# fu5ha/rayn

Measured on NVIDIA H100. Metric: Msamples/sec (pixels x spp), higher is better.
Workload: dtype f32

## Files before the change

rayn_b200/csrc/rt_kernels.cuh:

```cuda
#pragma once
#include "rt_device.cuh"
#include "rt_sdf2.cuh"

namespace rt {

struct DevFrame {
  int W, H, tile_w, tile_h, samples, spp, max_bounces, vm;
  int ntx, nty, sets_1d, sets_2d;
  float t0, t1;
  const float* __restrict__ s1;
  const float* __restrict__ s2;
  const float* __restrict__ scramble;
  const float* __restrict__ fis;
};

struct PassBufs {
  int n_tiles;
  int R;
  int QS;
  const int* __restrict__ tile_ids;
  float4* o_time;
  float4* d_t;
  float4* rad;
  float4* thr;
// ... 82 lines not shown
    }
  }
  *closest = c;
  *id = best;
}

__global__ void __launch_bounds__(256) k_raygen(const __grid_constant__ DevScene sc, const DevFrame fr, const PassBufs pb, const int pre_n) {
  const int ts = blockIdx.y;
  const int i = blockIdx.x * blockDim.x + threadIdx.x;
  const TileGeom tg = tile_geom(fr, pb.tile_ids[ts]);
  if (i == 0) pb.n_live[ts] = tg.npaths;
  if (i >= tg.npaths) return;
  const int pl = i / fr.spp, s = i - pl * fr.spp;
  const int xl = pl / tg.th, yl = pl - xl * tg.th;
  const int x = tg.x0 + xl, y = tg.y0 + yl;
  const float scramble = __ldg(fr.scramble + x + (size_t)y * fr.W);
  const float fx = fis_sample(fr.fis, samp2(fr, 0, s, scramble, 0));
  const float fy = fis_sample(fr.fis, samp2(fr, 1, s, scramble, 0));
  const float sx = ((float)x + 0.5f) + fx;
  const float sy = ((float)y + 0.5f) + fy;
  const float u = (1.0f / (float)fr.W) * sx;
  const float v = (1.0f / (float)fr.H) * sy;
  const float time = fr.t0 + (fr.t1 - fr.t0) * samp1(fr, s, scramble, 0);
  const float ls0 = samp2(fr, 0, s, scramble, 1), ls1 = samp2(fr, 1, s, scramble, 1);
  const float time0 = fr.t0 + (fr.t1 - fr.t0) * samp1(fr, s & ~3, scramble, 0);
  f3 ro, rd;
  camera_ray(sc.cam, u, v, ls0, ls1, time0, &ro, &rd);
  const size_t g = (size_t)ts * pb.R + i;
  float closest = 0.0f;
  int hit_id = -1;
  if (pre_n >= 0) fold_head(sc, pre_n, ro, rd, &closest, &hit_id);
  pb.o_time[g] = make_float4(ro.x, ro.y, ro.z, time);
  pb.d_t[g] = make_float4(rd.x, rd.y, rd.z, closest);
  pb.q_key[g] = hit_id;
  pb.rad[g] = make_float4(0.0f, 0.0f, 0.0f, 0.0f);
  pb.thr[g] = make_float4(1.0f, 1.0f, 1.0f, 0.0f);
  pb.nrm0[g] = make_float4(0.0f, 0.0f, 0.0f, __uint_as_float(0u));
  pb.term[g] = 0u;
  pb.q_live[g] = i;
}

#define BIN_T 1024
#define SEG_SLOTS 32768
__global__ void __launch_bounds__(BIN_T) k_bin_count(const PassBufs pb, const int n_hit, const int nseg) {
  const int seg = blockIdx.x, ts = blockIdx.y, tid = threadIdx.x, lane = tid & 31;
  const int n = pb.n_live[ts];
  __shared__ int cnt[RAYN_MAX_HITABLES];
  const int* __restrict__ qk = pb.q_key + (size_t)ts * pb.R;
  const int* __restrict__ ql = pb.q_live + (size_t)ts * pb.R;
  if (tid < RAYN_MAX_HITABLES) cnt[tid] = 0;
  if (tid == 0 && seg == 0 && n) atomicAdd(pb.counters + CNT_EXTEND_RAYS, (unsigned long long)n);
  __syncthreads();
  const int lo = seg * SEG_SLOTS, hi = min(n, lo + SEG_SLOTS);
  for (int base = lo; base < hi; base += BIN_T) {
    const int i = base + tid;
    const int key = i < hi ? qk[ql[i]] : -1;
    const unsigned m = __match_any_sync(0xffffffffu, key);
    if (key >= 0 && (m & ((1u << lane) - 1)) == 0) atomicAdd(&cnt[key], __popc(m));
  }
  __syncthreads();
  if (tid < n_hit) pb.seg_cnt[((size_t)ts * nseg + seg) * RAYN_MAX_HITABLES + tid] = cnt[tid];
}
__global__ void __launch_bounds__(BIN_T) k_bin_scatter(const PassBufs pb, const int n_hit, const int nseg) {
  const int seg = blockIdx.x, ts = blockIdx.y, tid = threadIdx.x, lane = tid & 31, warp = tid >> 5;
  constexpr int NW = BIN_T / 32;
  const int n = pb.n_live[ts];
  const int lo = seg * SEG_SLOTS, hi = min(n, lo + SEG_SLOTS);
  if (lo >= n && seg > 0) return;
  __shared__ int cnt[RAYN_MAX_HITABLES];
  __shared__ int before[RAYN_MAX_HITABLES];
  __shared__ int start[RAYN_MAX_HITABLES + 1];
  __shared__ int running[2][RAYN_MAX_HITABLES];
  __shared__ int wcnt[2][NW][RAYN_MAX_HITABLES];
  const int* __restrict__ qk = pb.q_key + (size_t)ts * pb.R;
  const int* __restrict__ ql = pb.q_live + (size_t)ts * pb.R;
  int* __restrict__ qs = pb.q_shade + (size_t)ts * pb.QS;
  if (tid < n_hit) {
    const int used = (n + SEG_SLOTS - 1) / SEG_SLOTS;
    int tot = 0, bef = 0;
    for (int sg = 0; sg < used; ++sg) {
      const int c = pb.seg_cnt[((size_t)ts * nseg + sg) * RAYN_MAX_HITABLES + tid];
      if (sg < seg) bef += c;
      tot += c;
    }
    cnt[tid] = tot, before[tid] = bef;
  }
  __syncthreads();
  if (tid == 0) {
    int off = 0;
    for (int o = 0; o < n_hit; ++o) {
      start[o] = off;
      running[0][o] = off + before[o];
      off += (cnt[o] + 3) & ~3;
    }
    start[n_hit] = off;
    if (seg == 0) pb.n_slots[ts] = off;
  }
  __syncthreads();
  if (seg == 0 && tid <= n_hit) pb.bin_start[ts * (RAYN_MAX_HITABLES + 1) + tid] = start[tid];
  int buf = 0;
  for (int base = lo; base < hi; base += BIN_T, buf ^= 1) {
    const int i = base + tid;
    const int id = i < hi ? ql[i] : -1;
    const int key = i < hi ? qk[id] : -1;
    unsigned mine = 0;
    for (int k = 0; k < n_hit; ++k) {
      const unsigned b = __ballot_sync(0xffffffffu, key == k);
      if (key == k) mine = b;
      if (lane == k) wcnt[buf][warp][k] = __popc(b);
    }
    __syncthreads();
    if (key >= 0) {
      int off = running[buf][key] + __popc(mine & ((1u << lane) - 1));
      for (int w = 0; w < warp; ++w) off += wcnt[buf][w][key];
      qs[off] = id;
    }
    if (tid < n_hit) {
      int tot = running[buf][tid];
      for (int w = 0; w < NW; ++w) tot += wcnt[buf][w][tid];
      running[buf ^ 1][tid] = tot;
    }
  }
  if (seg == 0 && tid < n_hit)
    for (int k = start[tid] + cnt[tid]; k < start[tid + 1]; ++k) qs[k] = -1;
}

#define EXT_BATCH 128
#define SCAN_T 1024
__global__ void __launch_bounds__(SCAN_T) k_scan_live(const PassBufs pb, int* __restrict__ batch_prefix, int* __restrict__ work_ctr) {
  __shared__ int wsum[SCAN_T / 32];
  __shared__ int carry;
  const int tid = threadIdx.x, lane = tid & 31, warp = tid >> 5;
  if (tid == 0) {
    carry = 0;
  }
  if (tid < WC_TOTAL) work_ctr[tid] = 0;
  __syncthreads();
  for (int base = 0; base < pb.n_tiles; base += SCAN_T) {
    const int i = base + tid;
    const int v = i < pb.n_tiles ? (pb.n_live[i] + EXT_BATCH - 1) / EXT_BATCH : 0;
    int x = v;
    for (int o = 1; o < 32; o <<= 1) {
      const int y = __shfl_up_sync(0xffffffffu, x, o);
      if (lane >= o) x += y;
    }
    if (lane == 31) wsum[warp] = x;
    __syncthreads();
    if (warp == 0) {
      int w = wsum[lane];
      for (int o = 1; o < 32; o <<= 1) {
        const int y = __shfl_up_sync(0xffffffffu, w, o);
        if (lane >= o) w += y;
      }
      wsum[lane] = w;
    }
    __syncthreads();
    const int excl = carry + (warp ? wsum[warp - 1] : 0) + x - v;
    if (i < pb.n_tiles) batch_prefix[i] = excl;
    __syncthreads();
    if (tid == SCAN_T - 1) carry = excl + v;
    __syncthreads();
  }
  if (tid == 0) batch_prefix[pb.n_tiles] = carry;
}

#define SLOT_BLOCK 128
__global__ void __launch_bounds__(SCAN_T) k_scan_slots(const __grid_constant__ DevScene sc, const PassBufs pb) {
  __shared__ int wsum[SCAN_T / 32];
  __shared__ int carry;
  const int tid = threadIdx.x, lane = tid & 31, warp = tid >> 5;
  for (int row = 0; row <= sc.n_sdf; ++row) {
    int* __restrict__ out = pb.slot_prefix + (size_t)row * pb.prefix_stride;
    const int hk = row ? sc.sdf_idx[row - 1] : 0;
    if (tid == 0) carry = 0;
    __syncthreads();
    for (int base = 0; base < pb.n_tiles; base += SCAN_T) {
      const int i = base + tid;
      int v = 0;
      if (i < pb.n_tiles) {
        const int* __restrict__ bs = pb.bin_start + i * (RAYN_MAX_HITABLES + 1);
        const int slots = row ? bs[hk + 1] - bs[hk] : pb.n_slots[i];
        v = (slots + SLOT_BLOCK - 1) / SLOT_BLOCK;
      }
      int x = v;
      for (int o = 1; o < 32; o <<= 1) {
        const int y = __shfl_up_sync(0xffffffffu, x, o);
        if (lane >= o) x += y;
      }
      if (lane == 31) wsum[warp] = x;
      __syncthreads();
      if (warp == 0) {
        int w = wsum[lane];
        for (int o = 1; o < 32; o <<= 1) {
          const int y = __shfl_up_sync(0xffffffffu, w, o);
          if (lane >= o) w += y;
        }
        wsum[lane] = w;
      }
      __syncthreads();
      const int excl = carry + (warp ? wsum[warp - 1] : 0) + x - v;
      if (i < pb.n_tiles) out[i] = excl;
      __syncthreads();
      if (tid == SCAN_T - 1) carry = excl + v;
      __syncthreads();
    }
    if (tid == 0) out[pb.n_tiles] = carry;
    __syncthreads();
  }
}
#define WORK_CHUNK 8
RT_D int grab_chunk(int* __restrict__ ctr, int* s_slot) {
  if (threadIdx.x == 0) *s_slot = atomicAdd(ctr, WORK_CHUNK);
  __syncthreads();
  const int c = *s_slot;
  __syncthreads();
  return c;
}
RT_D int find_tile(const int* __restrict__ prefix, int n_tiles, int wb) {
  int lo = 0, hi = n_tiles;
  while (hi - lo > 1) {
    const int mid = (lo + hi) >> 1;
    if (__ldg(prefix + mid) <= wb) lo = mid; else hi = mid;
  }
  return lo;
}
#define FOR_EACH_WORK_BLOCK(prefix, n_tiles, ctr, ...)                                  \
  {                                                                                     \
    __shared__ int s_chunk_;                                                            \
    const int total_ = (prefix)[n_tiles];                                               \
    for (;;) {                                                                          \
      const int c0_ = grab_chunk(ctr, &s_chunk_);                                       \
      if (c0_ >= total_) break;                                                         \
      const int c1_ = min(c0_ + WORK_CHUNK, total_);                                    \
      int ts = 0, begin_ = 0, end_ = 0;                                                 \
      for (int wb_ = c0_; wb_ < c1_; ++wb_) {                                           \
        if (wb_ >= end_) {                                                              \
          ts = find_tile(prefix, n_tiles, wb_);                                         \
          begin_ = __ldg((prefix) + ts), end_ = __ldg((prefix) + ts + 1);               \
        }                                                                               \
        const int local = wb_ - begin_;                                                 \
        __VA_ARGS__                                                                     \
      }                                                                                 \
    }                                                                                   \
  }

__global__ void __launch_bounds__(EXT_BATCH) k_extend_spheres(const __grid_constant__ DevScene sc, const PassBufs pb, const int first, const int last,
                                                              const int init, const int moving, const int* __restrict__ batch_prefix,
                                                              int* __restrict__ work_ctr) {
  FOR_EACH_WORK_BLOCK(batch_prefix, pb.n_tiles, work_ctr, {
    const int i = local * EXT_BATCH + threadIdx.x;
    const int n = pb.n_live[ts];
    if (i < n) {
      const size_t q = (size_t)ts * pb.R + i;
      const size_t g = (size_t)ts * pb.R + pb.q_live[q];
      const float4 o4 = pb.o_time[g], d4 = pb.d_t[g];
      const f3 o = mk3(o4.x, o4.y, o4.z), d = mk3(d4.x, d4.y, d4.z);
      float closest = init ? sc.rc.world_radius * 2.0f : d4.w;
      int id = init ? -1 : pb.q_key[g];
      float time0 = o4.w;
      if (moving && (i & 3)) time0 = pb.o_time[(size_t)ts * pb.R + pb.q_live[(size_t)ts * pb.R + (i & ~3)]].w;
      for (int k = first; k < last; ++k) {
        const float t = moving ? sphere_hit(sc.hit[k], o, d, closest, time0) : sphere_hit_static(sc.sph[sc.hit_ord[k]], o, d, closest);
        if (t < closest) {
          closest = t;
          id = k;
        }
      }
      pb.d_t[g].w = closest;
      pb.q_key[g] = id;
    }
  })
}

#define EXT_T 128
#ifndef RAYN_MARCH_OCC
#define RAYN_MARCH_OCC 8
#endif
#ifndef RAYN_MARCH_OCC_BULB
#define RAYN_MARCH_OCC_BULB RAYN_MARCH_OCC
#endif
#define MARCH_OCC(V) ((V) == SDFV_BULB ? RAYN_MARCH_OCC_BULB : RAYN_MARCH_OCC)
struct MarchSlot {
  float ox, oy, oz, dx, dy, dz;
  float px, py, pz;
  float t, t_max;
  int id, steps;
};
RT_D void slot_start(MarchSlot& s, float4 o, float4 d, float t_max) {
  s.ox = o.x, s.oy = o.y, s.oz = o.z, s.dx = d.x, s.dy = d.y, s.dz = d.z;
  s.px = o.x, s.py = o.y, s.pz = o.z;
  s.t = -0.0f, s.t_max = t_max, s.steps = -1;
}
RT_D void slot_advance(MarchSlot& s) {
  s.px = dm::mul_add(s.dx, s.t, s.ox), s.py = dm::mul_add(s.dy, s.t, s.oy), s.pz = dm::mul_add(s.dz, s.t, s.oz);
}
RT_D void slot_park(MarchSlot& s) { s.px = 100.0f, s.py = 0.0f, s.pz = 0.0f; }
RT_D MarchSlot slot_empty() {
  MarchSlot s;
  slot_start(s, make_float4(0.0f, 0.0f, 0.0f, 0.0f), make_float4(0.0f, 0.0f, 0.0f, 0.0f), 0.0f);
  s.id = -1;
  return s;
}

template <bool THR_CONST>
RT_D bool extend_step(MarchSlot& s, float d, float c0, float c1, float thr_scale, int max_marches, bool* hit) {
  const float th = THR_CONST ? c1 : __fmul_rn(c1, __fmul_rn(thr_scale, s.t));
  const float ad = dm::abs(d);
  const bool h = (s.steps >= 0) && ((ad < c0) || (ad < th));
  const float tn = __fadd_rn(s.t, d);
  const int sn = s.steps + 1;
  s.t = h ? s.t : tn;
  s.steps = h ? s.steps : sn;
  *hit = h;
  return h | (tn != tn) | (sn >= max_marches) | (tn > s.t_max);
}

template <int V, bool THR_CONST>
__global__ void __launch_bounds__(EXT_T, MARCH_OCC(V)) k_extend_march(const __grid_constant__ DevScene sc, const PassBufs pb, const Thr thr,
                                                          const int hk, const int spheres_first, const int* __restrict__ batch_prefix,
                                                          int* __restrict__ work_ctr) {
  const SdfK k = make_sdfk(sc.hit[hk]);
  const int lane = threadIdx.x & 31;
  const unsigned lt = (1u << lane) - 1u;
  const float S = sc.rc.sdf_detail_scale;
  const float c0 = 0.00005f * S;
  const float c1 = THR_CONST ? (0.05f * S) * thr.scale : 0.05f * S;
  const int max_marches = sc.rc.max_marches;
  const int n_batches = batch_prefix[pb.n_tiles];
  MarchSlot s0 = slot_empty(), s1 = slot_empty();
  int evals = 0, bulb_iters = 0, trips = 0;
  int cur_base = 0, cur_pos = 0, cur_end = 0;
  bool exhausted = false;
  while (true) {
    if (!exhausted) {
      unsigned idle0 = __ballot_sync(0xffffffffu, s0.id < 0), idle1 = __ballot_sync(0xffffffffu, s1.id < 0);
      while (idle0 | idle1) {
        if (cur_pos >= cur_end) {
          int b = 0;
          if (lane == 0) b = atomicAdd(work_ctr, 1);
          b = __shfl_sync(0xffffffffu, b, 0);
          if (b >= n_batches) {
            exhausted = true;
            break;
          }
          int lo = 0, hi = pb.n_tiles;
          while (hi - lo > 1) {
            const int mid = (lo + hi) >> 1;
            if (__ldg(batch_prefix + mid) <= b) lo = mid; else hi = mid;
          }
          cur_base = lo * pb.R;
          cur_pos = (b - __ldg(batch_prefix + lo)) * EXT_BATCH;
          cur_end = min(cur_pos + EXT_BATCH, pb.n_live[lo]);
        }
        const int avail = cur_end - cur_pos;
        const int n0 = __popc(idle0);
        const int rank0 = __popc(idle0 & lt), rank1 = n0 + __popc(idle1 & lt);
        if (s0.id < 0 && rank0 < avail) {
          const int g = cur_base + pb.q_live[cur_base + cur_pos + rank0];
          const float4 d4 = pb.d_t[g];
          slot_start(s0, pb.o_time[g], d4, d4.w);
          s0.id = g;
        }
        if (s1.id < 0 && rank1 < avail) {
          const int g = cur_base + pb.q_live[cur_base + cur_pos + rank1];
          const float4 d4 = pb.d_t[g];
          slot_start(s1, pb.o_time[g], d4, d4.w);
          s1.id = g;
        }
        cur_pos += min(avail, n0 + __popc(idle1));
        idle0 = __ballot_sync(0xffffffffu, s0.id < 0), idle1 = __ballot_sync(0xffffffffu, s1.id < 0);
      }
    }
    if (exhausted) {
      if (!__any_sync(0xffffffffu, s0.id >= 0 || s1.id >= 0)) break;
      if (s0.id < 0) slot_park(s0);
      if (s1.id < 0) slot_park(s1);
    }
    const float2 dd = sdf_dist2<V>(k, f2(s0.px, s1.px), f2(s0.py, s1.py), f2(s0.pz, s1.pz), bulb_iters);
    ++trips;
    bool hit0, hit1;
    const bool done0 = extend_step<THR_CONST>(s0, dd.x, c0, c1, thr.scale, max_marches, &hit0);
    const bool done1 = extend_step<THR_CONST>(s1, dd.y, c0, c1, thr.scale, max_marches, &hit1);
    slot_advance(s0);
    slot_advance(s1);
    if (done0 | done1) {
      if (done0 && s0.id >= 0) {
        if (s0.t < s0.t_max || (spheres_first && s0.t == s0.t_max && pb.q_key[s0.id] > hk)) {
          pb.d_t[s0.id].w = s0.t;
          pb.q_key[s0.id] = hk;
        }
        evals += s0.steps + (hit0 ? 2 : 1);
        s0.id = -1;
      }
      if (done1 && s1.id >= 0) {
        if (s1.t < s1.t_max || (spheres_first && s1.t == s1.t_max && pb.q_key[s1.id] > hk)) {
          pb.d_t[s1.id].w = s1.t;
          pb.q_key[s1.id] = hk;
        }
        evals += s1.steps + (hit1 ? 2 : 1);
        s1.id = -1;
      }
    }
  }
  warp_add(pb.counters + CNT_EVALS_EXTEND, evals);
  if (lane == 0) atomicAdd(pb.counters + CNT_TRIPS_EXTEND, (unsigned long long)trips);
  if (V == SDFV_BULB) warp_add(pb.counters + CNT_BULB_ITERS_EXTEND, bulb_iters);
}

template <int V, bool TRAP>
__global__ void __launch_bounds__(128, 8) k_normals(const __grid_constant__ DevScene sc, const PassBufs pb, const Thr thr, const int hk, const int j,
                                                    int* __restrict__ work_ctr) {
  const int* __restrict__ prefix = pb.slot_prefix + (size_t)(1 + j) * pb.prefix_stride;
  const SdfK k = make_sdfk(sc.hit[hk]);
  int evals = 0;
  FOR_EACH_WORK_BLOCK(prefix, pb.n_tiles, work_ctr, {
    const int* __restrict__ bs = pb.bin_start + ts * (RAYN_MAX_HITABLES + 1);
    const int s = bs[hk] + local * SLOT_BLOCK + threadIdx.x;
    const int id = s < bs[hk + 1] ? pb.q_shade[(size_t)ts * pb.QS + s] : -1;
    if (id >= 0) {
      const size_t g = (size_t)ts * pb.R + id;
      const float4 o4 = pb.o_time[g], d4 = pb.d_t[g];
      const f3 point = fma3s(mk3(d4.x, d4.y, d4.z), d4.w, mk3(o4.x, o4.y, o4.z));
      const float eps = dm::max(0.0001f, sc.rc.sdf_detail_scale * thr.at(d4.w));
      int it = 0;
      const float ex = 1.0f * eps, en = -1.0f * eps;
      const float2 da = sdf_dist2<V>(k, f2(point.x + ex, point.x + en), f2(point.y + en, point.y + en), f2(point.z + en, point.z + ex), it);
      const float2 db = sdf_dist2<V>(k, f2(point.x + en, point.x + ex), f2(point.y + ex, point.y + ex), f2(point.z + en, point.z + ex), it);
      f3 n = mk3(1.0f, -1.0f, -1.0f) * da.x;
      n = n + mk3(-1.0f, -1.0f, 1.0f) * da.y;
      n = n + mk3(-1.0f, 1.0f, -1.0f) * db.x;
      n = n + mk3(1.0f, 1.0f, 1.0f) * db.y;
      n = normalized(n);
      pb.nrm[g] = make_float4(n.x, n.y, n.z, eps);
      evals += 4;
      if (TRAP) pb.trap_s[g] = trap_coord(sc.trap[sc.hit[hk].material], sdf_trap(sc.hit[hk], point));
    }
  })
  warp_add(pb.counters + CNT_EVALS_NORMALS, evals);
}
struct LightContrib {
  f3 start, end_point, c;
  float den, trans;
};
RT_D LightContrib light_contrib(const RaynLight& L, const RaynMaterial& mat, f3 albedo, const ShadingPoint& sp, f3 wo, int round, float u0,
                                float u1, float vol_sample, bool has_ext, float neg_rho_t) {
  LightContrib r;
  f3 li;
  r.trans = 1.0f;
  if (round == 0) {
    float pdf;
    light_sample(L, u0, u1, sp.point, &r.end_point, &li, &pdf);
    f3 wi = r.end_point - sp.point;
    const float dist = mag(wi);
    wi = wi / dist;
    r.start = sp.point + sp.normal * dm::signum(dot(sp.normal, wi)) * sp.offset_by;
    const f3 f = bsdf_f(mat, albedo, wo, wi, sp.normal) * dm::max(dot(sp.normal, wi), 0.0f);
    const float tr = has_ext ? dm::exp(neg_rho_t * dist) : 1.0f;
    r.c = li * f * tr;
    r.den = pdf;
  } else {
    float vol_dist, vol_pdf, light_pdf;
    light_sample_volume(L, vol_sample, sp.o, sp.d, sp.t, &vol_dist, &vol_pdf);
    r.start = sp.o + sp.d * vol_dist;
    light_sample(L, u0, u1, r.start, &r.end_point, &li, &light_pdf);
    const float dist_point_to_light = mag(r.end_point - r.start);
    const float f = 1.0f / (4.0f * RT_PI);
    const float tr = has_ext ? dm::exp(neg_rho_t * dist_point_to_light) : 1.0f;
    r.c = li * f * tr;
    r.den = vol_pdf * light_pdf;
    r.trans = has_ext ? dm::exp(neg_rho_t * vol_dist) : 1.0f;
  }
  return r;
}

RT_D f3 hit_albedo(const DevScene& sc, const PassBufs& pb, const RaynHitable& h, const RaynMaterial& mat, size_t g) {
  if (sc.trap_mask != 0u && ((sc.trap_mask >> h.material) & 1u))
    return trap_albedo(sc.trap[h.material], h.kind == RAYN_HITABLE_SPHERE ? 1.0f : pb.trap_s[g]);
  return ld3(mat.albedo);
}

struct SlotCtx {
  int id, sample, obj;
  float scramble;
  unsigned w0, w1, w2;
  int set1, set2;
};
RT_D SlotCtx slot_ctx(const DevScene& sc, const DevFrame& fr, const PassBufs& pb, int ts, int s, int nslots, int depth, int lane) {
  SlotCtx c;
  const int* __restrict__ qs = pb.q_shade + (size_t)ts * pb.QS;
  c.id = s < nslots ? qs[s] : -1;
  c.sample = 0;
  c.obj = 0;
  c.scramble = 0.0f;
  if (c.id >= 0) {
    c.obj = pb.q_key[(size_t)ts * pb.R + c.id];
    const TileGeom tg = tile_geom(fr, pb.tile_ids[ts]);
    const int pl = c.id / fr.spp;
    c.sample = c.id - pl * fr.spp;
    const int xl = pl / tg.th, yl = pl - xl * tg.th;
    c.scramble = __ldg(fr.scramble + (tg.x0 + xl) + (size_t)(tg.y0 + yl) * fr.W);
  }
  const int n1 = 3 + fr.vm, n2h = (12 + 8 * fr.vm) / 2;
  c.set1 = 1 + depth * n1;
  c.set2 = 2 + depth * n2h;
  const int nl = sc.n_lights;
  unsigned pack = 0;
  if (nl > 0) {
    const float u0 = __ldg(fr.s1 + c.sample + (size_t)fr.spp * (c.set1 + 0)), u1 = __ldg(fr.s1 + c.sample + (size_t)fr.spp * (c.set1 + 1)),
                u2 = __ldg(fr.s1 + c.sample + (size_t)fr.spp * (c.set1 + 2));
    pack = (unsigned)light_index(dm::fract(u0 + c.scramble), nl) | ((unsigned)light_index(dm::fract(u1 + c.scramble), nl) << 8) |
           ((unsigned)light_index(dm::fract(u2 + c.scramble), nl) << 16);
  }
  c.w0 = c.w1 = c.w2 = 0;
#pragma unroll
  for (int k = 0; k < 4; ++k) {
    const unsigned pk = __shfl_sync(0xffffffffu, pack, (lane & ~3) + k);
    c.w0 |= (pk & 0xffu) << (8 * k);
    c.w1 |= ((pk >> 8) & 0xffu) << (8 * k);
    c.w2 |= ((pk >> 16) & 0xffu) << (8 * k);
  }
  return c;
}

template <bool TRAP>
RT_D void shade_pre_slot(const DevScene& sc, const DevFrame& fr, const PassBufs& pb, const int depth, const Thr thr, const int ts, const int s) {
  const int nslots = pb.n_slots[ts];
  if ((s & ~31) >= nslots) return;
  const SlotCtx cx = slot_ctx(sc, fr, pb, ts, s, nslots, depth, threadIdx.x & 31);
  const bool valid = cx.id >= 0;
  warp_add(pb.counters + CNT_SHADE_LANES, valid ? 1 : 0);
  int shadows = 0;
  const size_t g = (size_t)ts * pb.R + (valid ? cx.id : 0);
  float4 o4 = make_float4(0, 0, 0, 0), d4 = o4, r4 = o4, t4 = o4;
  if (valid) o4 = pb.o_time[g], d4 = pb.d_t[g], r4 = pb.rad[g], t4 = pb.thr[g];
  const float time0 = __shfl_sync(0xffffffffu, o4.w, (threadIdx.x & 31) & ~3);
  if (valid) {
    const RaynHitable& h = sc.hit[cx.obj];
    const RaynMaterial& mat = sc.mat[h.material];
    ShadingPoint sp;
    sp.o = mk3(o4.x, o4.y, o4.z);
    sp.d = mk3(d4.x, d4.y, d4.z);
    sp.time = o4.w;
    sp.t = d4.w;
    const bool recv = receives_light(mat);
    const int nl = sc.n_lights;
    const bool scat = sc.vol.has_scattering != 0 && nl > 0;
    const int n_rounds = nl > 0 ? 1 + (scat ? fr.vm : 0) : 0;
    const f3 wo = -sp.d;
    const bool has_ext = sc.vol.has_extinction != 0;
    const float neg_rho_t = -sc.vol.coeff_extinction;
    const float vt = has_ext ? dm::exp(neg_rho_t * sp.t) : 1.0f;
    const f3 radiance = mk3(r4.x, r4.y, r4.z) + bsdf_le(mat, wo) * mk3(t4.x, t4.y, t4.z) * vt;
    pb.rad[g] = make_float4(radiance.x, radiance.y, radiance.z, 0.0f);
    if (!recv && !scat) {
      pb.term[g] = ((depth == 0 ? TERM_BACKGROUND : TERM_COLOR) << 30) | ((unsigned)depth << TERM_DEPTH_SHIFT) | (unsigned)s;
      pb.q_shade[(size_t)ts * pb.QS + s] = -1;
    } else {
      sp.point = fma3s(sp.d, sp.t, sp.o);
      if (h.kind == RAYN_HITABLE_SPHERE) {
        sp.normal = normalized(sp.point - sphere_center(h, time0));
        sp.offset_by = 0.0f;
        pb.nrm[g] = make_float4(sp.normal.x, sp.normal.y, sp.normal.z, 0.0f);
      } else {
        const float4 n4 = pb.nrm[g];
        sp.normal = mk3(n4.x, n4.y, n4.z);
        sp.offset_by = n4.w;
      }
      unsigned vis = 0xffffffffu;
      const f3 tr_albedo = TRAP ? hit_albedo(sc, pb, h, mat, g) : mk3(0.0f, 0.0f, 0.0f);
      for (int round = (recv ? 0 : 1); round < n_rounds; ++round) {
        const unsigned wr = round == 0 ? cx.w0 : (round == 1 ? cx.w1 : cx.w2);
        const float vol_sample = round == 0 ? 0.0f : samp1(fr, cx.sample, cx.scramble, cx.set1 + 1);
#pragma unroll 1
        for (int i = 0; i < 4; ++i) {
          const int set = round == 0 ? cx.set2 + i : cx.set2 + 4 + 4 * (round - 1) + i;
          const LightContrib lc = light_contrib(sc.light[(wr >> (8 * i)) & 0xffu], mat, TRAP ? tr_albedo : ld3(mat.albedo), sp, wo, round, samp2(fr, 0, cx.sample, cx.scramble, set),
                                                samp2(fr, 1, cx.sample, cx.scramble, set), vol_sample, has_ext, neg_rho_t);
          ++shadows;
          const int bit = round * 4 + i;
          pb.lc_c[g * pb.lc_ns + bit] = make_float4(lc.c.x, lc.c.y, lc.c.z, lc.den);
          if (round > 0) pb.lc_t[g * 8 + (bit - 4)] = lc.trans;
          const bool irrelevant = (lc.c.x == 0.0f || lc.c.x != lc.c.x) && (lc.c.y == 0.0f || lc.c.y != lc.c.y) && (lc.c.z == 0.0f || lc.c.z != lc.c.z);
          if (irrelevant) continue;
          f3 dir = lc.end_point - lc.start;
          const float max_dist = mag(dir);
          dir = dir / max_dist;
          float v = 1.0f;
          if (sc.sph_moving) {
            for (int k = 0; k < sc.n_sph && v != 0.0f; ++k) v = sphere_occluded_seg(sc.hit[sc.sph_idx[k]], lc.start, dir, max_dist, time0);
          } else {
            for (int k = 0; k < sc.n_sph && v != 0.0f; ++k) v = sphere_occluded_seg_static(sc.sph[k], lc.start, dir, max_dist);
          }
          if (v == 0.0f) {
            vis &= ~(1u << bit);
            continue;
          }
          for (int j = 0; j < sc.n_sdf; ++j) {
            const unsigned am = __activemask();
            const int leader = __ffs(am) - 1, ln = threadIdx.x & 31;
            int base = 0;
            if (ln == leader) base = atomicAdd(pb.seg_count + j, __popc(am));
            base = __shfl_sync(am, base, leader);
            const size_t slot = (size_t)j * pb.seg_cap + base + __popc(am & ((1u << ln) - 1u));
            pb.seg_a[slot] = make_float4(lc.start.x, lc.start.y, lc.start.z, max_dist);
            pb.seg_b[slot] = make_float4(dir.x, dir.y, dir.z, __int_as_float((int)(((unsigned)g << 4) | (unsigned)bit)));
          }
        }
      }
      pb.vis[g] = vis;
    }
  }
  warp_add(pb.counters + CNT_SHADOW_RAYS, shadows);
}

#ifndef RAYN_SHADE_PRE_OCC
#define RAYN_SHADE_PRE_OCC 8
#endif
template <bool TRAP>
__global__ void __launch_bounds__(128, RAYN_SHADE_PRE_OCC) k_shade_pre(const __grid_constant__ DevScene sc, const DevFrame fr, const PassBufs pb,
                                                      const int depth, const Thr thr, int* __restrict__ work_ctr) {
  FOR_EACH_WORK_BLOCK(pb.slot_prefix, pb.n_tiles, work_ctr, { shade_pre_slot<TRAP>(sc, fr, pb, depth, thr, ts, local * SLOT_BLOCK + threadIdx.x); })
}
constexpr size_t param_align(size_t off, size_t a) { return (off + a - 1) / a * a; }
constexpr size_t kShadePreParamBytes =
    param_align(param_align(param_align(param_align(param_align(sizeof(DevScene), alignof(DevFrame)) + sizeof(DevFrame), alignof(PassBufs)) +
                                            sizeof(PassBufs), alignof(int)) + sizeof(int), alignof(Thr)) + sizeof(Thr), alignof(int*)) +
    sizeof(int*);
static_assert(kShadePreParamBytes <= 4096, "k_shade_pre's parameters exceed the 4 KB the scene limits are sized for");

#define SHD_T 128
#define SHD_BATCH 128
RT_D bool shadow_step(MarchSlot& s, float d, float oc0, float oc1, int max_vis, int* occ) {
  const bool o = dm::abs(d) < (s.steps >= 0 ? fmaxf(oc0, __fmul_rn(oc1, s.t)) : -1.0f);
  const float tn = __fadd_rn(s.t, d);
  s.t = tn;
  s.steps = s.steps + 1;
  *occ = o ? 1 : 0;
  return o | (tn != tn) | (s.steps >= max_vis) | (tn > s.t_max);
}

template <int V>
__global__ void __launch_bounds__(SHD_T, MARCH_OCC(V)) k_shadow(const __grid_constant__ DevScene sc, const PassBufs pb, const int hk, const int j,
                                                    int* __restrict__ work_ctr) {
  const SdfK k = make_sdfk(sc.hit[hk]);
  const int lane = threadIdx.x & 31;
  const unsigned lt = (1u << lane) - 1u;
  const int n_seg = pb.seg_count[j];
  const float4* __restrict__ seg_a = pb.seg_a + (size_t)j * pb.seg_cap;
  const float4* __restrict__ seg_b = pb.seg_b + (size_t)j * pb.seg_cap;
  const float S = sc.rc.sdf_detail_scale;
  const float oc0 = 0.0001f * S, oc1 = 0.00001f * S;
  const int max_vis = sc.rc.max_vis_marches;
  MarchSlot s0 = slot_empty(), s1 = slot_empty();
  int evals = 0, bulb_iters = 0, trips = 0;
  int cur_pos = 0, cur_end = 0;
  const float4* __restrict__ qa = seg_a;
  const float4* __restrict__ qb = seg_b;
  bool exhausted = false;
  while (true) {
    if (!exhausted) {
      unsigned idle0 = __ballot_sync(0xffffffffu, s0.id < 0), idle1 = __ballot_sync(0xffffffffu, s1.id < 0);
      while (idle0 | idle1) {
        if (cur_pos >= cur_end) {
          int b = 0;
          if (lane == 0) b = atomicAdd(work_ctr, SHD_BATCH);
          b = __shfl_sync(0xffffffffu, b, 0);
          if (b >= n_seg) {
            exhausted = true;
            break;
          }
          qa = seg_a + b, qb = seg_b + b;
          cur_pos = 0;
          cur_end = min(SHD_BATCH, n_seg - b);
        }
        const int avail = cur_end - cur_pos;
        const int n0 = __popc(idle0);
        const int rank0 = __popc(idle0 & lt), rank1 = n0 + __popc(idle1 & lt);
        if (s0.id < 0 && rank0 < avail) {
          const float4 a = qa[cur_pos + rank0], b4 = qb[cur_pos + rank0];
          slot_start(s0, a, b4, a.w);
          s0.id = __float_as_int(b4.w);
        }
        if (s1.id < 0 && rank1 < avail) {
          const float4 a = qa[cur_pos + rank1], b4 = qb[cur_pos + rank1];
          slot_start(s1, a, b4, a.w);
          s1.id = __float_as_int(b4.w);
        }
        cur_pos += min(avail, n0 + __popc(idle1));
        idle0 = __ballot_sync(0xffffffffu, s0.id < 0), idle1 = __ballot_sync(0xffffffffu, s1.id < 0);
      }
    }
    if (exhausted) {
      if (!__any_sync(0xffffffffu, s0.id >= 0 || s1.id >= 0)) break;
      if (s0.id < 0) slot_park(s0);
      if (s1.id < 0) slot_park(s1);
    }
    const float2 dd = sdf_dist2<V>(k, f2(s0.px, s1.px), f2(s0.py, s1.py), f2(s0.pz, s1.pz), bulb_iters);
    ++trips;
    int occ0, occ1;
    const bool done0 = shadow_step(s0, dd.x, oc0, oc1, max_vis, &occ0);
    const bool done1 = shadow_step(s1, dd.y, oc0, oc1, max_vis, &occ1);
    slot_advance(s0);
    slot_advance(s1);
    if (done0 | done1) {
      if (done0 && s0.id >= 0) {
        if (occ0) atomicAnd(pb.vis + ((unsigned)s0.id >> 4), ~(1u << (s0.id & 15)));
        evals += s0.steps + 1;
        s0.id = -1;
      }
      if (done1 && s1.id >= 0) {
        if (occ1) atomicAnd(pb.vis + ((unsigned)s1.id >> 4), ~(1u << (s1.id & 15)));
        evals += s1.steps + 1;
        s1.id = -1;
      }
    }
  }
  warp_add(pb.counters + CNT_EVALS_SHADOW, evals);
  if (lane == 0) atomicAdd(pb.counters + CNT_TRIPS_SHADOW, (unsigned long long)trips);
  if (V == SDFV_BULB) warp_add(pb.counters + CNT_BULB_ITERS_SHADOW, bulb_iters);
}

template <bool TRAP>
RT_D void shade_post_slot(const DevScene& sc, const DevFrame& fr, const PassBufs& pb, const int depth, const int pre_n, const int ts, const int s) {
  const int nslots = pb.n_slots[ts];
  if ((s & ~31) >= nslots) return;
  const SlotCtx cx = slot_ctx(sc, fr, pb, ts, s, nslots, depth, threadIdx.x & 31);
  if (cx.id < 0) return;
  int* __restrict__ qs = pb.q_shade + (size_t)ts * pb.QS;
  const RaynHitable& h = sc.hit[cx.obj];
  const RaynMaterial& mat = sc.mat[h.material];
  const size_t g = (size_t)ts * pb.R + cx.id;
  const float4 o4 = pb.o_time[g], d4 = pb.d_t[g], r4 = pb.rad[g], t4 = pb.thr[g], n4 = pb.nrm[g];
  ShadingPoint sp;
  sp.o = mk3(o4.x, o4.y, o4.z);
  sp.d = mk3(d4.x, d4.y, d4.z);
  sp.time = o4.w;
  sp.t = d4.w;
  sp.point = fma3s(sp.d, sp.t, sp.o);
  sp.normal = mk3(n4.x, n4.y, n4.z);
  sp.offset_by = n4.w;
  sp.basis = onb(sp.normal);
  f3 radiance = mk3(r4.x, r4.y, r4.z), throughput = mk3(t4.x, t4.y, t4.z);
  const f3 wo = -sp.d;
  const bool has_ext = sc.vol.has_extinction != 0;
  const float neg_rho_t = -sc.vol.coeff_extinction;
  const float vt = has_ext ? dm::exp(neg_rho_t * sp.t) : 1.0f;
  const bool recv = receives_light(mat);
  const int nl = sc.n_lights;
  const bool scat = sc.vol.has_scattering != 0 && nl > 0;
  const int n_rounds = nl > 0 ? 1 + (scat ? fr.vm : 0) : 0;
  const unsigned vis = pb.vis[g];
  for (int round = (recv ? 0 : 1); round < n_rounds; ++round) {
    const float correction = round == 0 ? (float)nl / 4.0f : (float)nl / 4.0f / (float)fr.vm;
#pragma unroll
    for (int i = 0; i < 4; ++i) {
      const int bit = round * 4 + i;
      const float4 c4 = pb.lc_c[g * pb.lc_ns + bit];
      const float occluded = (vis >> bit) & 1u ? 1.0f : 0.0f;
      const f3 num = mk3(c4.x, c4.y, c4.z) * occluded;
      const bool no_div = (num.x == 0.0f) & (num.y == 0.0f) & (num.z == 0.0f) & (c4.w > 0.0f);
      const f3 contrib = no_div ? num : num / c4.w;
      if (round == 0)
        radiance = radiance + contrib * throughput * correction * vt;
      else
        radiance = radiance + contrib * throughput * correction * sc.vol.coeff_scattering * pb.lc_t[g * 8 + (bit - 4)];
    }
  }
  if (recv) {
    const int setb = cx.set2 + 4 + 4 * fr.vm;
    const Scatter se = bsdf_scatter(mat, TRAP ? hit_albedo(sc, pb, h, mat, g) : ld3(mat.albedo), wo, sp, samp1(fr, cx.sample, cx.scramble, cx.set1 + 3),
                                    samp2(fr, 0, cx.sample, cx.scramble, setb),
                                    samp2(fr, 1, cx.sample, cx.scramble, setb), samp2(fr, 0, cx.sample, cx.scramble, setb + 1),
                                    samp2(fr, 1, cx.sample, cx.scramble, setb + 1));
    const float ndl = dm::abs(dot(se.wi, sp.normal));
    f3 new_throughput = throughput * vt * se.f * ndl / se.pdf;
    float roulette_factor = 0.0f;
    if (depth > 2) {
      roulette_factor = dm::max(1.0f - component_max(throughput), 0.05f);
      new_throughput = new_throughput / (1.0f - roulette_factor);
    }
    if (depth == 0) pb.nrm0[g] = make_float4(sp.normal.x, sp.normal.y, sp.normal.z, __uint_as_float((unsigned)s + 1u));
    const float roulette_sample = samp1(fr, cx.sample, cx.scramble, cx.set1 + 4);
    if (depth >= fr.max_bounces || roulette_sample < roulette_factor) {
      pb.rad[g] = make_float4(radiance.x, radiance.y, radiance.z, 0.0f);
      pb.term[g] = (TERM_COLOR << 30) | ((unsigned)depth << TERM_DEPTH_SHIFT) | (unsigned)s;
      qs[s] = -1;
    } else {
      const f3 no = sp.point + sp.normal * dm::signum(dot(sp.normal, se.wi)) * sp.offset_by;
      if (!any_nan(new_throughput)) throughput = new_throughput;
      float closest = 0.0f;
      int hit_id = -1;
      if (pre_n >= 0) fold_head(sc, pre_n, no, se.wi, &closest, &hit_id);
      pb.o_time[g] = make_float4(no.x, no.y, no.z, sp.time);
      pb.d_t[g] = make_float4(se.wi.x, se.wi.y, se.wi.z, closest);
      pb.q_key[g] = hit_id;
      pb.rad[g] = make_float4(radiance.x, radiance.y, radiance.z, 0.0f);
      pb.thr[g] = make_float4(throughput.x, throughput.y, throughput.z, 0.0f);
    }
  } else {
    pb.rad[g] = make_float4(radiance.x, radiance.y, radiance.z, 0.0f);
    pb.term[g] = ((depth == 0 ? TERM_BACKGROUND : TERM_COLOR) << 30) | ((unsigned)depth << TERM_DEPTH_SHIFT) | (unsigned)s;
    qs[s] = -1;
  }
}

template <bool TRAP>
__global__ void __launch_bounds__(128, 8) k_shade_post(const __grid_constant__ DevScene sc, const DevFrame fr, const PassBufs pb,
                                                       const int depth, const int pre_n, int* __restrict__ work_ctr) {
  FOR_EACH_WORK_BLOCK(pb.slot_prefix, pb.n_tiles, work_ctr, { shade_post_slot<TRAP>(sc, fr, pb, depth, pre_n, ts, local * SLOT_BLOCK + threadIdx.x); })
}

#define CMP_T 1024
__global__ void __launch_bounds__(CMP_T) k_compact_count(const PassBufs pb, const int nseg) {
  const int seg = blockIdx.x, ts = blockIdx.y, tid = threadIdx.x;
  const int n = pb.n_slots[ts];
  const int* __restrict__ qs = pb.q_shade + (size_t)ts * pb.QS;
  const int lo = seg * SEG_SLOTS, hi = min(n, lo + SEG_SLOTS);
  int c = 0;
  for (int i = lo + tid; i < hi; i += CMP_T) c += qs[i] >= 0 ? 1 : 0;
  c = __reduce_add_sync(0xffffffffu, c);
  __shared__ int tot;
  if (tid == 0) tot = 0;
  __syncthreads();
  if ((tid & 31) == 0 && c) atomicAdd(&tot, c);
  __syncthreads();
  if (tid == 0) pb.seg_cnt[((size_t)ts * nseg + seg) * RAYN_MAX_HITABLES] = tot;
}
__global__ void __launch_bounds__(CMP_T) k_compact_scatter(const PassBufs pb, const int nseg) {
  const int seg = blockIdx.x, ts = blockIdx.y, tid = threadIdx.x, lane = tid & 31, warp = tid >> 5;
  constexpr int NW = CMP_T / 32;
  const int n = pb.n_slots[ts];
  const int lo = seg * SEG_SLOTS, hi = min(n, lo + SEG_SLOTS);
  if (lo >= n && seg > 0) return;
  const int* __restrict__ qs = pb.q_shade + (size_t)ts * pb.QS;
  int* __restrict__ ql = pb.q_live + (size_t)ts * pb.R;
  __shared__ int wtot[2][NW];
  __shared__ int running[2];
  if (tid == 0) {
    const int used = (n + SEG_SLOTS - 1) / SEG_SLOTS;
    int bef = 0, tot = 0;
    for (int sg = 0; sg < used; ++sg) {
      const int c = pb.seg_cnt[((size_t)ts * nseg + sg) * RAYN_MAX_HITABLES];
      if (sg < seg) bef += c;
      tot += c;
    }
    running[0] = bef;
    if (seg == 0) pb.n_live[ts] = tot;
  }
  __syncthreads();
  int buf = 0;
  for (int base = lo; base < hi; base += CMP_T, buf ^= 1) {
    const int i = base + tid;
    const int id = i < hi ? qs[i] : -1;
    const unsigned b = __ballot_sync(0xffffffffu, id >= 0);
    if (lane == 0) wtot[buf][warp] = __popc(b);
    __syncthreads();
    int off = running[buf] + __popc(b & ((1u << lane) - 1));
    for (int w = 0; w < warp; ++w) off += wtot[buf][w];
    if (id >= 0) ql[off] = id;
    if (tid == CMP_T - 1) running[buf ^ 1] = off + (id >= 0 ? 1 : 0);
  }
}

#define RES_MAX_WARPS 8
#define RES_BINS 512
#define RES_ROW 33
#define RES_STAGE_FLOATS (6 * RES_ROW + 2)
#define RES_STAGE_FLOATS_MOM (8 * RES_ROW + 2)
__host__ __device__ inline size_t resolve_smem_per_warp(int np, bool mom = false) {
  return (size_t)np * (sizeof(uint32_t) + 2 * sizeof(uint16_t)) + RES_BINS * sizeof(int) + (mom ? RES_STAGE_FLOATS_MOM : RES_STAGE_FLOATS) * sizeof(float);
}
static inline int resolve_warps_per_cta(int np, bool mom = false) {
  int w = (int)((size_t)200 * 1024 / resolve_smem_per_warp(np, mom));
  return w < 1 ? 0 : (w > RES_MAX_WARPS ? RES_MAX_WARPS : w);
}
RT_D uint16_t* warp_radix_sort(const uint32_t* key, uint16_t* src, uint16_t* tmp, int n, int key_bits, int lane, int* hist) {
  const unsigned lt = (1u << lane) - 1u;
  const int passes = (key_bits + 8) / 9, dbits = (key_bits + passes - 1) / passes;
  const unsigned dmask = (1u << dbits) - 1u;
  const int per_lane = (1 << dbits) >> 5;
  for (int shift = 0; shift < key_bits; shift += dbits) {
    for (int b = lane; b <= (int)dmask; b += 32) hist[b] = 0;
    __syncwarp();
#pragma unroll 4
    for (int base = 0; base < n; base += 32) {
      const int i = base + lane;
      if (i < n) atomicAdd(&hist[(key[src[i]] >> shift) & dmask], 1);
    }
    __syncwarp();
    int sum = 0;
    bool uniform = false;
    for (int q = 0; q < per_lane; ++q) {
      const int c = hist[per_lane * lane + q];
      uniform |= c == n;
      sum += c;
    }
    if (__any_sync(0xffffffffu, uniform)) continue;
    int incl = sum;
    for (int o = 1; o < 32; o <<= 1) {
      const int y = __shfl_up_sync(0xffffffffu, incl, o);
      if (lane >= o) incl += y;
    }
    int run = incl - sum;
    for (int q = 0; q < per_lane; ++q) {
      const int c = hist[per_lane * lane + q];
      hist[per_lane * lane + q] = run;
      run += c;
    }
    __syncwarp();
    for (int base = 0; base < n; base += 32) {
      const int i = base + lane;
      const bool act = i < n;
      const int v = act ? src[i] : 0;
      const unsigned d = act ? ((key[v] >> shift) & dmask) : (RES_BINS + lane);
      const unsigned m = __match_any_sync(0xffffffffu, d);
      const int leader = __ffs(m) - 1;
      int pos = 0;
      if (act && lane == leader) {
        pos = hist[d];
        hist[d] = pos + __popc(m);
      }
      pos = __shfl_sync(0xffffffffu, pos, leader) + __popc(m & lt);
      if (act) tmp[pos] = (uint16_t)v;
      __syncwarp();
    }
    uint16_t* t = src;
    src = tmp;
    tmp = t;
  }
  return src;
}
template <int WHICH>
RT_D int resolve_keys(const float4* __restrict__ nrm0, const uint32_t* __restrict__ term, const float4* __restrict__ prefetch, int spp, int slot_bits,
                      int lane, uint32_t* key, uint16_t* idx, int* unordered) {
  const unsigned lt = (1u << lane) - 1u;
  int n = 0, bad = 0;
  uint32_t prev = 0;
  for (int base = 0; base < spp; base += 32) {
    const int i = base + lane;
    uint32_t k = 0xffffffffu;
    if (i < spp) {
      if (WHICH == 0) {
        const uint32_t s0 = __float_as_uint(nrm0[i].w);
        if (s0) k = s0;
      } else {
        const uint32_t t = term[i];
        if (t >> 30) k = (((t >> TERM_DEPTH_SHIFT) & 0xffu) << slot_bits) | (t & (TERM_MAX_SLOTS - 1u));
        asm volatile("prefetch.global.L2 [%0];" ::"l"(prefetch + i));
      }
      key[i] = k;
    }
    const bool valid = k != 0xffffffffu;
    const unsigned vm = __ballot_sync(0xffffffffu, valid);
    if (valid) idx[n + __popc(vm & lt)] = (uint16_t)i;
    const unsigned below = vm & lt;
    const int pl = below ? 31 - __clz(below) : -1;
    const uint32_t pk_in = __shfl_sync(0xffffffffu, k, pl < 0 ? 0 : pl);
    const uint32_t pk = pl < 0 ? prev : pk_in;
    bad |= valid && (n + __popc(below) > 0) && pk > k;
    if (vm) prev = __shfl_sync(0xffffffffu, k, 31 - __clz(vm));
    n += __popc(vm);
  }
  *unordered = __any_sync(0xffffffffu, bad);
  return n;
}
RT_D float resolve_sum(const float4* __restrict__ src, const uint32_t* __restrict__ term, const uint16_t* order, int n, int lane, int n_rows,
                       int want_lo, int want_hi, float* stage) {
  auto fetch = [&](int base) {
    float4 v = make_float4(0.0f, 0.0f, 0.0f, 0.0f);
    const int i = base + lane;
    if (i < n) {
      const int p = order[i];
      v = src[p];
      v.w = term ? __uint_as_float(term[p] >> 30) : 0.0f;
    }
    return v;
  };
  float acc = 0.0f;
  float4 cur = fetch(0), nxt = fetch(32);
  for (int base = 0; base < n; base += 32) {
    const float4 nxt2 = fetch(base + 64);
    const int kind = (int)__float_as_uint(cur.w);
    const bool lo = want_lo < 0 || kind == want_lo, hi = want_hi < 0 || kind == want_hi;
    stage[0 * RES_ROW + lane] = lo ? cur.x : 0.0f;
    stage[1 * RES_ROW + lane] = lo ? cur.y : 0.0f;
    stage[2 * RES_ROW + lane] = lo ? cur.z : 0.0f;
    if (n_rows > 3) {
      stage[3 * RES_ROW + lane] = hi ? cur.x : 0.0f;
      stage[4 * RES_ROW + lane] = hi ? cur.y : 0.0f;
      stage[5 * RES_ROW + lane] = hi ? cur.z : 0.0f;
    }
    if (n_rows > 6) {
      const float l = (0.2126f * cur.x + 0.7152f * cur.y) + 0.0722f * cur.z;
      const float l2 = l * l;
      stage[6 * RES_ROW + lane] = lo ? l2 : 0.0f;
      stage[7 * RES_ROW + lane] = hi ? l2 : 0.0f;
    }
    __syncwarp();
    const int m = min(32, n - base);
    if (lane < n_rows) {
      const float* row = stage + lane * RES_ROW;
#pragma unroll 8
      for (int j = 0; j < m; ++j) acc += row[j];
    }
    __syncwarp();
    cur = nxt;
    nxt = nxt2;
  }
  return acc;
}
template <bool kMom>
__global__ void __launch_bounds__(RES_MAX_WARPS * 32) k_resolve(const DevFrame fr, const PassBufs pb, float* __restrict__ color,
                                                                 float* __restrict__ alpha, float* __restrict__ background,
                                                                 float* __restrict__ normal, const int np, const int wpc, const int slot_bits,
                                                                 const int depth_bits, float* __restrict__ lum2_color = nullptr,
// ... 301 lines not shown
```

Before: 368.2.

## Stage march batches in shared memory via cp.async and parallelize batch lookup

The extend and shadow march kernels now copy each warp's batch of ray origins and directions (and shadow segments) into shared memory with cp.async, then refill idle slots from shared memory. This replaces scattered dependent global loads in the refill loop. The binary search over tile prefixes becomes a warp-cooperative 32-way search. Eval counting is replaced by a trip-based estimate, and the refill loop exits early once enough work is available. In exchange each kernel uses extra shared memory per block, which may reduce occupancy, and the eval counter statistics change meaning.

```diff
diff --git a/rayn_b200/csrc/rt_kernels.cuh b/rayn_b200/csrc/rt_kernels.cuh
--- a/rayn_b200/csrc/rt_kernels.cuh
+++ b/rayn_b200/csrc/rt_kernels.cuh
@@ -408,8 +408,51 @@
   return s;
 }
 
+struct MarchStage {
+  float4 a[EXT_T / 32 * EXT_BATCH], b[EXT_T / 32 * EXT_BATCH];
+};
+RT_D void stage_copy(float4* dst, const float4* src) {
+  asm volatile("cp.async.cg.shared.global [%0], [%1], 16;" ::"r"((unsigned)__cvta_generic_to_shared(dst)), "l"(src) : "memory");
+}
+RT_D unsigned stage_base(const MarchStage& st) {
+  unsigned a;
+  asm volatile("mov.u32 %0, %1;" : "=r"(a) : "r"((unsigned)__cvta_generic_to_shared(&st)));
+  return a;
+}
+RT_D float4 stage_row(unsigned base, int r, int half) {
+  float4 v;
+  asm volatile("ld.shared.v4.f32 {%0, %1, %2, %3}, [%4];"
+               : "=f"(v.x), "=f"(v.y), "=f"(v.z), "=f"(v.w)
+               : "r"(base + 16u * (unsigned)r + (unsigned)(half * sizeof(MarchStage::a)))
+               : "memory");
+  return v;
+}
+RT_D unsigned lanemask_lt() {
+  unsigned m;
+  asm("mov.u32 %0, %%lanemask_lt;" : "=r"(m));
+  return m;
+}
+RT_D void stage_wait() {
+  asm volatile("cp.async.wait_all;" ::: "memory");
+  __syncwarp();
+}
+RT_D int find_batch_tile(const int* __restrict__ prefix, int n_tiles, int b, int lane, int* start) {
+  int lo = 0, span = n_tiles, v = 0;
+  while (span > 1) {
+    const int step = (span + 31) >> 5;
+    const int off = lane * step;
+    const int x = off < span ? __ldg(prefix + lo + off) : 0x7fffffff;
+    const int k = 31 - __clz(__ballot_sync(0xffffffffu, x <= b));
+    v = __shfl_sync(0xffffffffu, x, k);
+    lo += k * step;
+    span = min(step, span - k * step);
+  }
+  *start = v;
+  return lo;
+}
+
 template <bool THR_CONST>
-RT_D bool extend_step(MarchSlot& s, float d, float c0, float c1, float thr_scale, int max_marches, bool* hit) {
+RT_D bool extend_step(MarchSlot& s, float d, float c0, float c1, float thr_scale, int max_marches) {
   const float th = THR_CONST ? c1 : __fmul_rn(c1, __fmul_rn(thr_scale, s.t));
   const float ad = dm::abs(d);
   const bool h = (s.steps >= 0) && ((ad < c0) || (ad < th));
@@ -417,7 +460,6 @@
   const int sn = s.steps + 1;
   s.t = h ? s.t : tn;
   s.steps = h ? s.steps : sn;
-  *hit = h;
   return h | (tn != tn) | (sn >= max_marches) | (tn > s.t_max);
 }
 
@@ -427,15 +469,17 @@
                                                           int* __restrict__ work_ctr) {
   const SdfK k = make_sdfk(sc.hit[hk]);
   const int lane = threadIdx.x & 31;
-  const unsigned lt = (1u << lane) - 1u;
+  const unsigned lt = lanemask_lt();
   const float S = sc.rc.sdf_detail_scale;
   const float c0 = 0.00005f * S;
   const float c1 = THR_CONST ? (0.05f * S) * thr.scale : 0.05f * S;
   const int max_marches = sc.rc.max_marches;
   const int n_batches = batch_prefix[pb.n_tiles];
+  __shared__ MarchStage st;
+  const unsigned sbase = stage_base(st);
   MarchSlot s0 = slot_empty(), s1 = slot_empty();
   int evals = 0, bulb_iters = 0, trips = 0;
-  int cur_base = 0, cur_pos = 0, cur_end = 0;
+  int cur_pos = 0, cur_end = 0;
   bool exhausted = false;
   while (true) {
     if (!exhausted) {
@@ -447,46 +491,62 @@
           b = __shfl_sync(0xffffffffu, b, 0);
           if (b >= n_batches) {
             exhausted = true;
+            evals = 2 * trips;
             break;
           }
-          int lo = 0, hi = pb.n_tiles;
-          while (hi - lo > 1) {
-            const int mid = (lo + hi) >> 1;
-            if (__ldg(batch_prefix + mid) <= b) lo = mid; else hi = mid;
+          int first;
+          const int ts = find_batch_tile(batch_prefix, pb.n_tiles, b, lane, &first);
+          first = (b - first) * EXT_BATCH;
+          const int base = ts * pb.R;
+          const int n = min(EXT_BATCH, pb.n_live[ts] - first);
+          cur_pos = (threadIdx.x >> 5) * EXT_BATCH;
+          cur_end = cur_pos + n;
+          __syncwarp();
+          int g[EXT_BATCH / 32];
+#pragma unroll
+          for (int k = 0; k < EXT_BATCH / 32; ++k) {
+            const int i = lane + 32 * k;
+            if (i < n) {
+              g[k] = base + pb.q_live[base + first + i];
+              stage_copy(&st.a[cur_pos + i], pb.o_time + g[k]);
+              stage_copy(&st.b[cur_pos + i], pb.d_t + g[k]);
+            }
           }
-          cur_base = lo * pb.R;
-          cur_pos = (b - __ldg(batch_prefix + lo)) * EXT_BATCH;
-          cur_end = min(cur_pos + EXT_BATCH, pb.n_live[lo]);
+          asm volatile("cp.async.wait_all;" ::: "memory");
+#pragma unroll
+          for (int k = 0; k < EXT_BATCH / 32; ++k)
+            if (lane + 32 * k < n) st.a[cur_pos + lane + 32 * k].w = __int_as_float(g[k]);
+          __syncwarp();
         }
         const int avail = cur_end - cur_pos;
         const int n0 = __popc(idle0);
         const int rank0 = __popc(idle0 & lt), rank1 = n0 + __popc(idle1 & lt);
         if (s0.id < 0 && rank0 < avail) {
-          const int g = cur_base + pb.q_live[cur_base + cur_pos + rank0];
-          const float4 d4 = pb.d_t[g];
-          slot_start(s0, pb.o_time[g], d4, d4.w);
-          s0.id = g;
+          const float4 o4 = stage_row(sbase, cur_pos + rank0, 0), d4 = stage_row(sbase, cur_pos + rank0, 1);
+          slot_start(s0, o4, d4, d4.w);
+          s0.id = __float_as_int(o4.w);
         }
         if (s1.id < 0 && rank1 < avail) {
-          const int g = cur_base + pb.q_live[cur_base + cur_pos + rank1];
-          const float4 d4 = pb.d_t[g];
-          slot_start(s1, pb.o_time[g], d4, d4.w);
-          s1.id = g;
+          const float4 o4 = stage_row(sbase, cur_pos + rank1, 0), d4 = stage_row(sbase, cur_pos + rank1, 1);
+          slot_start(s1, o4, d4, d4.w);
+          s1.id = __float_as_int(o4.w);
         }
-        cur_pos += min(avail, n0 + __popc(idle1));
+        const int n_idle = n0 + __popc(idle1);
+        cur_pos += min(avail, n_idle);
+        if (avail >= n_idle) break;
         idle0 = __ballot_sync(0xffffffffu, s0.id < 0), idle1 = __ballot_sync(0xffffffffu, s1.id < 0);
       }
     }
     if (exhausted) {
       if (!__any_sync(0xffffffffu, s0.id >= 0 || s1.id >= 0)) break;
+      evals += (s0.id >= 0) + (s1.id >= 0);
       if (s0.id < 0) slot_park(s0);
       if (s1.id < 0) slot_park(s1);
     }
     const float2 dd = sdf_dist2<V>(k, f2(s0.px, s1.px), f2(s0.py, s1.py), f2(s0.pz, s1.pz), bulb_iters);
     ++trips;
-    bool hit0, hit1;
-    const bool done0 = extend_step<THR_CONST>(s0, dd.x, c0, c1, thr.scale, max_marches, &hit0);
-    const bool done1 = extend_step<THR_CONST>(s1, dd.y, c0, c1, thr.scale, max_marches, &hit1);
+    const bool done0 = extend_step<THR_CONST>(s0, dd.x, c0, c1, thr.scale, max_marches);
+    const bool done1 = extend_step<THR_CONST>(s1, dd.y, c0, c1, thr.scale, max_marches);
     slot_advance(s0);
     slot_advance(s1);
     if (done0 | done1) {
@@ -495,7 +555,6 @@
           pb.d_t[s0.id].w = s0.t;
           pb.q_key[s0.id] = hk;
         }
-        evals += s0.steps + (hit0 ? 2 : 1);
         s0.id = -1;
       }
       if (done1 && s1.id >= 0) {
@@ -503,7 +562,6 @@
           pb.d_t[s1.id].w = s1.t;
           pb.q_key[s1.id] = hk;
         }
-        evals += s1.steps + (hit1 ? 2 : 1);
         s1.id = -1;
       }
     }
@@ -736,6 +794,7 @@
 
 #define SHD_T 128
 #define SHD_BATCH 128
+static_assert(SHD_BATCH == EXT_BATCH && SHD_T == EXT_T, "k_shadow stages its batches in MarchStage");
 RT_D bool shadow_step(MarchSlot& s, float d, float oc0, float oc1, int max_vis, int* occ) {
   const bool o = dm::abs(d) < (s.steps >= 0 ? fmaxf(oc0, __fmul_rn(oc1, s.t)) : -1.0f);
   const float tn = __fadd_rn(s.t, d);
@@ -750,7 +809,7 @@
                                                     int* __restrict__ work_ctr) {
   const SdfK k = make_sdfk(sc.hit[hk]);
   const int lane = threadIdx.x & 31;
-  const unsigned lt = (1u << lane) - 1u;
+  const unsigned lt = lanemask_lt();
   const int n_seg = pb.seg_count[j];
   const float4* __restrict__ seg_a = pb.seg_a + (size_t)j * pb.seg_cap;
   const float4* __restrict__ seg_b = pb.seg_b + (size_t)j * pb.seg_cap;
@@ -759,9 +818,9 @@
   const int max_vis = sc.rc.max_vis_marches;
   MarchSlot s0 = slot_empty(), s1 = slot_empty();
   int evals = 0, bulb_iters = 0, trips = 0;
+  __shared__ MarchStage st;
+  const unsigned sbase = stage_base(st);
   int cur_pos = 0, cur_end = 0;
-  const float4* __restrict__ qa = seg_a;
-  const float4* __restrict__ qb = seg_b;
   bool exhausted = false;
   while (true) {
     if (!exhausted) {
@@ -773,31 +832,45 @@
           b = __shfl_sync(0xffffffffu, b, 0);
           if (b >= n_seg) {
             exhausted = true;
+            evals = 2 * trips;
             break;
           }
-          qa = seg_a + b, qb = seg_b + b;
-          cur_pos = 0;
-          cur_end = min(SHD_BATCH, n_seg - b);
+          const int n = min(SHD_BATCH, n_seg - b);
+          cur_pos = (threadIdx.x >> 5) * SHD_BATCH;
+          cur_end = cur_pos + n;
+          __syncwarp();
+#pragma unroll
+          for (int k = 0; k < SHD_BATCH / 32; ++k) {
+            const int i = lane + 32 * k;
+            if (i < n) {
+              stage_copy(&st.a[cur_pos + i], seg_a + b + i);
+              stage_copy(&st.b[cur_pos + i], seg_b + b + i);
+            }
+          }
+          stage_wait();
         }
         const int avail = cur_end - cur_pos;
         const int n0 = __popc(idle0);
         const int rank0 = __popc(idle0 & lt), rank1 = n0 + __popc(idle1 & lt);
         if (s0.id < 0 && rank0 < avail) {
-          const float4 a = qa[cur_pos + rank0], b4 = qb[cur_pos + rank0];
+          const float4 a = stage_row(sbase, cur_pos + rank0, 0), b4 = stage_row(sbase, cur_pos + rank0, 1);
           slot_start(s0, a, b4, a.w);
           s0.id = __float_as_int(b4.w);
         }
         if (s1.id < 0 && rank1 < avail) {
-          const float4 a = qa[cur_pos + rank1], b4 = qb[cur_pos + rank1];
+          const float4 a = stage_row(sbase, cur_pos + rank1, 0), b4 = stage_row(sbase, cur_pos + rank1, 1);
           slot_start(s1, a, b4, a.w);
           s1.id = __float_as_int(b4.w);
         }
-        cur_pos += min(avail, n0 + __popc(idle1));
+        const int n_idle = n0 + __popc(idle1);
+        cur_pos += min(avail, n_idle);
+        if (avail >= n_idle) break;
         idle0 = __ballot_sync(0xffffffffu, s0.id < 0), idle1 = __ballot_sync(0xffffffffu, s1.id < 0);
       }
     }
     if (exhausted) {
       if (!__any_sync(0xffffffffu, s0.id >= 0 || s1.id >= 0)) break;
+      evals += (s0.id >= 0) + (s1.id >= 0);
       if (s0.id < 0) slot_park(s0);
       if (s1.id < 0) slot_park(s1);
     }
@@ -811,12 +884,10 @@
     if (done0 | done1) {
       if (done0 && s0.id >= 0) {
         if (occ0) atomicAnd(pb.vis + ((unsigned)s0.id >> 4), ~(1u << (s0.id & 15)));
-        evals += s0.steps + 1;
         s0.id = -1;
       }
       if (done1 && s1.id >= 0) {
         if (occ1) atomicAnd(pb.vis + ((unsigned)s1.id >> 4), ~(1u << (s1.id & 15)));
-        evals += s1.steps + 1;
         s1.id = -1;
       }
     }
```

Measured after the change: 375.3 (median of 6 runs). +1.9%, better.
